# timlod/onset-fingerprinting

Hardware: AMD Instinct MI355X
Metric: frames/sec (1024-pt, hop 256, 48 kHz) detect+FFT+classify at 1/2/4/8 MI355X (higher is better)
Workload: dtype f32

## Files before the change

onset_fingerprinting_amd/csrc/ofp_detect.hip:

```cpp
#include <algorithm>
#include <cstdlib>
#include <cmath>
#include <cstring>
#include <new>
#include <vector>

#include "../../include/ofp_math.h"
#include "ofp_common.h"

#include "ofp_detector.h"

#define OFP_LATENCY_BOUND_KERNEL() __builtin_amdgcn_s_setprio(3)

namespace {

using ofp::align_up;
using ofp::cdiv;

typedef float v2f __attribute__((ext_vector_type(2)));

struct Geom {
    int64_t N;
    int64_t Nm;
    int64_t n_w;
// ... 44 lines not shown
        }
    };
    auto load = [&](float4 (&v)[PB4]) {
#pragma unroll
        for (int i = 0; i < PB4; ++i) v[i] = q[i];
        q += PB4;
        __builtin_amdgcn_sched_barrier(0);
    };
    auto run = [&](const float4 (&v)[PB4]) {
        batch(v);
        __builtin_amdgcn_sched_barrier(0);
    };
    float4 A[PB4], Bv[PB4];
    if (nb >= PB4) {
        load(A);
        nb -= PB4;
        while (nb >= 2 * PB4) {
            load(Bv); run(A);
            load(A); run(Bv);
            nb -= 2 * PB4;
        }
        run(A);
    }
    while (nb > 0) {
        const float4 v = *q++;
        one(v.x); one(v.y); one(v.z); one(v.w);
        --nb;
    }
    ip = reinterpret_cast<const float*>(q);
    for (int r = (int)(n & 3); r > 0; --r) one(*ip++);
}

constexpr int WL_PITCH = 36;
template <class F, class D>
__device__ __forceinline__ void walk_lines_to(const float* in0, const float* ip, int64_t n, F& f, float* tile, float* base, D&& dst_of) {
    const int lane = threadIdx.x & 63;
    const int64_t nb = n >> 5;
    int64_t nbmax = nb;
    for (int o = 32; o > 0; o >>= 1) nbmax = max(nbmax, __shfl_xor(nbmax, o));
    const float4* q = reinterpret_cast<const float4*>(ip);
    float4 A[8], Bv[8];
    auto load = [&](float4 (&v)[8], int64_t b) {
        const bool have = b < nb;
        const float4* const p = have ? q : reinterpret_cast<const float4*>(in0);
#pragma unroll
        for (int i = 0; i < 8; ++i) v[i] = p[i];
        q += have ? 8 : 0;
        __builtin_amdgcn_sched_barrier(0);
    };
    auto run = [&](const float4 (&v)[8], int64_t b) {
        const bool have = b < nb;
        if (have) {
#pragma unroll
            for (int i = 0; i < 8; ++i) {
                float4 o;
                o.x = f(v[i].x); o.y = f(v[i].y); o.z = f(v[i].z); o.w = f(v[i].w);
                *reinterpret_cast<float4*>(&tile[lane * WL_PITCH + 4 * i]) = o;
            }
        }
        __builtin_amdgcn_fence(__ATOMIC_RELEASE, "workgroup");
        __builtin_amdgcn_wave_barrier();
        __builtin_amdgcn_fence(__ATOMIC_ACQUIRE, "workgroup");
        const int64_t my = have ? dst_of(b) : -1;
        const unsigned long long hv = __ballot(my >= 0);
#pragma unroll
        for (int j = 0; j < 8; ++j) {
            const int owner = 8 * j + (lane >> 3);
            const int lo = __shfl((int)my, owner), hi = __shfl((int)(my >> 32), owner);
            if ((hv >> owner) & 1ull) {
                float* dst = base + (((int64_t)hi << 32) | (uint32_t)lo) + 4 * (lane & 7);
                *reinterpret_cast<float4*>(dst) = *reinterpret_cast<const float4*>(&tile[owner * WL_PITCH + 4 * (lane & 7)]);
            }
        }
        __builtin_amdgcn_wave_barrier();
        __builtin_amdgcn_sched_barrier(0);
    };
    load(A, 0);
    int64_t b = 0;
    for (; b + 1 < nbmax; b += 2) {
        load(Bv, b + 1); run(A, b);
        load(A, b + 2); run(Bv, b + 1);
    }
    if (b < nbmax) run(A, b);
}
template <class F>
__device__ __forceinline__ void walk_lines(const float* in0, const float* ip, float* base, int64_t off, int64_t n, F& f, float* tile) {
    walk_lines_to(in0, ip, n, f, tile, base, [off](int64_t b) { return off + 32 * b; });
}

template <int CH, int PB, bool EV, class F>
__device__ __forceinline__ void walk_il(const float* ip, int64_t n, int& rem, F& f) {
    auto one = [&](float x) {
        f(x);
        if (EV && rem >= 0) {
            if (rem == 0) f.event();
// ... 292 lines not shown
template <int W>
__device__ __forceinline__ bool chunk_pass_start(int pass, int64_t k, int64_t sidx, const uint32_t* end_prev,
                                                 uint32_t* end_next, uint32_t* used, bool has_dirty, uint8_t* dirty,
                                                 int* changed, uint32_t (&st)[W]) {
#pragma unroll
    for (int w = 0; w < W; ++w) st[w] = used[sidx + w];
    if (pass == 0) return true;
    uint32_t p[W];
    bool keep = k == 0;
    if (!keep) {
        keep = true;
#pragma unroll
        for (int w = 0; w < W; ++w) {
            p[w] = end_prev[sidx - 2 + w];
            keep = keep && p[w] == st[w];
        }
        if (has_dirty && *dirty != 0) keep = false;
    }
    if (keep) {
        keep_end<W>(end_prev, end_next, sidx);
        return false;
    }
    if (has_dirty) *dirty = 0;
#pragma unroll
    for (int w = 0; w < W; ++w) used[sidx + w] = st[w] = p[w];
    atomicAdd(changed, 1);
    return true;
}

struct ArArgs {
    Geom g;
    const float* xdb;
    float* dif;
    float fa, fr, sa, sr, floor_db;
    int64_t L, W, Wc, Wf, n_chunks;
    int64_t S;
    int lines;
    int through;
};
__device__ __forceinline__ bool chunk_walked(int64_t k, int64_t S, int64_t n_chunks) {
    return k + 1 < min((k / S) * S + S, n_chunks);
}

__global__ __launch_bounds__(64) void k_ar_coarse(ArArgs a, int64_t n_threads, uint32_t* __restrict__ used) {
    OFP_LATENCY_BOUND_KERNEL();
    const int64_t id = (int64_t)blockIdx.x * blockDim.x + threadIdx.x;
    if (id >= n_threads) return;
    const LaneAt ln = lane_planar(id, a.n_chunks, a.g.C);
    const int64_t ws = max<int64_t>(ln.k * a.L - a.W, 0);
    const float* xs = a.xdb + ln.chain * a.g.U;
    ArCoarse cs{a.floor_db, a.floor_db, a.fa, a.fr, a.sa, a.sr};
    if (ws > 0) {
        const int64_t t0 = max<int64_t>(ws - a.Wc, 0);
        if (t0 > 0) cs.yf = cs.ys = xs[t0];
        int norem = -1;
        walk<16, 0, false>(xs + t0, nullptr, ws - t0, norem, cs);
    }
    put_state(used, ln.sidx(a.n_chunks), cs.yf, cs.ys);
}

__global__ __launch_bounds__(64) void k_ar_sym_local(ArArgs a, int64_t n_waves, double* __restrict__ P) {
    OFP_LATENCY_BOUND_KERNEL();
    const int64_t id = blockIdx.x;
    if (id >= n_waves) return;
    const int lane = threadIdx.x;
    const int64_t j = id % a.n_chunks;
    const int64_t chain = id / a.n_chunks;
    const int64_t base = j * a.L;
    const int64_t len = min(a.L, a.g.U - base);
    const float* xs = a.xdb + chain * a.g.U + base;
    const double c = (double)a.sa, q = 1.0 - c;
    double q64 = 1.0, w = c;
    for (int i = 0; i < 64; ++i) {
        q64 *= q;
// ... 71 lines not shown
__global__ __launch_bounds__(64) void k_ar_warm2(ArArgs a, int64_t n_threads, uint32_t* __restrict__ used) {
    OFP_LATENCY_BOUND_KERNEL();
    const int64_t half = (n_threads + 63) / 64;
    const bool fast = blockIdx.x >= half;
    const int64_t id = ((int64_t)blockIdx.x - (fast ? half : 0)) * blockDim.x + threadIdx.x;
    if (id >= n_threads) return;
    const LaneAt ln = lane_planar(id, cdiv(a.n_chunks, a.S), a.g.C);
    const int64_t chain = ln.chain;
    const int64_t k0 = ln.k * a.S;
    const int64_t start = k0 * a.L;
    const float* xs = a.xdb + chain * a.g.U;
    int norem = -1;
    if (!fast) {
        const int64_t ws = max<int64_t>(start - a.W, 0);
        ArOne s{ofp_u2f(used[state_idx(chain, a.n_chunks, k0) + 1]), a.sa, a.sr};
        walk<8, 0, false>(xs + ws, nullptr, start - ws, norem, s);
        put_state(used, state_idx(chain, a.n_chunks, k0) + 1, s.y);
        for (int64_t k = k0 + 1; k < min(k0 + a.S, a.n_chunks); ++k) {
            walk<8, 0, false>(xs + (k - 1) * a.L, nullptr, a.L, norem, s);
            put_state(used, state_idx(chain, a.n_chunks, k) + 1, s.y);
        }
    } else {
        const int64_t ws = max<int64_t>(start - min(a.W, a.Wf), 0);
        ArOne s{a.floor_db, a.fa, a.fr};
        walk<8, 0, false>(xs + ws, nullptr, start - ws, norem, s);
        put_state(used, state_idx(chain, a.n_chunks, k0), s.y);
        for (int64_t k = k0 + 1; k < min(k0 + a.S, a.n_chunks); ++k) {
            walk<8, 0, false>(xs + (k - 1) * a.L, nullptr, a.L, norem, s);
            put_state(used, state_idx(chain, a.n_chunks, k), s.y);
        }
    }
}

template <bool LINES>
__global__ __launch_bounds__(64) void k_ar_warm_both(ArArgs a, int64_t n_threads, uint32_t* __restrict__ used,
                                                     uint32_t* __restrict__ end0) {
    OFP_LATENCY_BOUND_KERNEL();
    __shared__ float tile[LINES ? 64 * WL_PITCH : 1];
    const int64_t id = (int64_t)blockIdx.x * blockDim.x + threadIdx.x;
    const bool live = id < n_threads;
    if (!LINES && !live) return;
    const LaneAt ln = lane_planar(id, cdiv(a.n_chunks, a.S), a.g.C, live);
    const int64_t chain = ln.chain;
    const int64_t k0 = ln.k * a.S;
    const int64_t start = k0 * a.L;
    const float* xs = a.xdb + chain * a.g.U;
    int norem = -1;
    const int64_t ws = max<int64_t>(start - a.W, 0);
    const int64_t s0 = state_idx(chain, a.n_chunks, k0);
    ArStep s{a.floor_db, live ? ofp_u2f(used[s0 + 1]) : 0.0f, a.fa, a.fr, a.sa, a.sr};
    if (live) {
        walk<8, 0, false>(xs + ws, nullptr, start - ws, norem, s);
        put_state(used, s0, s.yf, s.ys);
    }
    float* os = a.dif + chain * a.g.U;
    if (LINES) {
        for (int64_t i = 1; i < a.S; ++i) {
            const int64_t k = k0 + i;
            const bool on = live && k < a.n_chunks;
            walk_lines(a.xdb, xs + (on ? (k - 1) * a.L : 0), a.dif, chain * a.g.U + (on ? (k - 1) * a.L : 0), on ? a.L : 0, s, tile);
            if (on) {
                put_state(used, state_idx(chain, a.n_chunks, k), s.yf, s.ys);
                put_state(end0, (chain * a.n_chunks + k - 1) * 2, s.yf, s.ys);
            }
        }
        return;
    }
    for (int64_t k = k0 + 1; k < min(k0 + a.S, a.n_chunks); ++k) {
        if (a.through) walk<8, 4, false>(xs + (k - 1) * a.L, os + (k - 1) * a.L, a.L, norem, s);
        else walk<8, 0, false>(xs + (k - 1) * a.L, nullptr, a.L, norem, s);
        put_state(used, state_idx(chain, a.n_chunks, k), s.yf, s.ys);
        if (a.through) put_state(end0, (chain * a.n_chunks + k - 1) * 2, s.yf, s.ys);
    }
}

template <bool LINES>
__global__ __launch_bounds__(64) void k_ar_chunk(ArArgs a, int pass, int64_t n_threads,
                                                 const uint32_t* __restrict__ end_prev,
                                                 uint32_t* __restrict__ end_next, uint32_t* __restrict__ used,
                                                 int* changed, const int* gate) {
    OFP_LATENCY_BOUND_KERNEL();
    if (gate && *gate == 0) return;
    __shared__ float tile[LINES ? 64 * WL_PITCH : 1];
    const int64_t id = (int64_t)blockIdx.x * blockDim.x + threadIdx.x;
    bool act = id < n_threads;
    const LaneAt ln = lane_planar(id, a.n_chunks, a.g.C, act);
    const int64_t k = ln.k, chain = ln.chain;
    const int64_t start = k * a.L;
    const int64_t end = min(start + a.L, a.g.U);
    const int64_t sidx = ln.sidx(a.n_chunks);
    if (act && pass == 0 && a.through && chunk_walked(k, a.S, a.n_chunks)) act = false;
    uint32_t st[2] = {0, 0};
    if (act) act = chunk_pass_start<2>(pass, k, sidx, end_prev, end_next, used, false, nullptr, changed, st);
    ArStep s{ofp_u2f(st[0]), ofp_u2f(st[1]), a.fa, a.fr, a.sa, a.sr};
    if (LINES) {
        if (!__any(act)) return;
        walk_lines(a.xdb, a.xdb + chain * a.g.U + start, a.dif, chain * a.g.U + start, act ? end - start : 0, s, tile);
    } else {
        if (!act) return;
        int norem = -1;
        walk<8, 4, false>(a.xdb + chain * a.g.U + start, a.dif + chain * a.g.U + start, end - start, norem, s);
    }
    if (act) put_state(end_next, sidx, s.yf, s.ys);
}

struct MmArgs {
    Geom g;
    const float* rel;
    const float* rel_il;
    const float* rel_warm;
    float* thr_mn;
    float* thr_mx;
    float alpha_min, alpha_max, ialpha_min, ialpha_max, minmin, min0, max0;
    int64_t nb, L, W, n_chunks;
    uint8_t* dirty;
    int64_t n_chains;
    int64_t S;
    int through;
};
constexpr int64_t MM_WARM_FULL = 12288;

__device__ __forceinline__ int64_t mm_block_end(const MmArgs& a, int64_t clip, int c, int C, int64_t start, int& rem) {
    const int64_t m = start - a.g.n_wb;
    int64_t j = 0;
    if (m >= 0) {
        j = m / a.g.B;
        rem = (int)(a.g.B - 1 - (m - j * a.g.B));
    } else {
        rem = (int)min<int64_t>(-m + a.g.B - 1, 0x7fffffff);
    }
// ... 1095 lines not shown
    const int64_t m0 = u0 - g.n_wb;
    if (vec && (m0 >= 0 || m0 + nt <= 0) && (reinterpret_cast<uintptr_t>(rel_out) & 15u) == 0) {
        if (m0 < 0 && !dstw) return;
        float4* d4 = reinterpret_cast<float4*>(m0 < 0 ? dstw + u0 * C : dst + m0 * C);
        const int lc = (C & (C - 1)) == 0 ? 31 - __clz(C) : -1;
        for (int i = threadIdx.x; i < (total >> 2); i += 256) {
            float o[4];
#pragma unroll
            for (int e = 0; e < 4; ++e) {
                const int j = 4 * i + e;
                const int t = lc >= 0 ? j >> lc : j / C, c = j - t * C;
                o[e] = tile[c * S + t];
            }
            d4[i] = make_float4(o[0], o[1], o[2], o[3]);
        }
        return;
    }
    for (int i = threadIdx.x; i < total; i += 256) {
        const int t = i / C, c = i - t * C;
        const int64_t m = u0 + t - g.n_wb;
        if (m >= 0) dst[m * C + c] = tile[c * S + t];
        else if (dstw) dstw[(u0 + t) * C + c] = tile[c * S + t];
    }
}

__global__ __launch_bounds__(256) void k_rel_out(Geom g, float* __restrict__ buf, float* __restrict__ rel_out,
                                                 float floor_db, int TU, uint32_t* __restrict__ sum_max,
                                                 uint32_t* __restrict__ sum_minv, int64_t nb, float* __restrict__ rel_warm,
                                                 int planar, int64_t n_tiles) {
    extern __shared__ float tile[];
    for (int64_t tx = blockIdx.x; tx < n_tiles; tx += gridDim.x) {
        rel_out_tile(g, buf, rel_out, floor_db, TU, sum_max, sum_minv, nb, rel_warm, planar, tx, tile);
        __syncthreads();
    }
}

struct ScanArgs {
    Geom g;
    const float* rel;
    const float* thr_mn;
    const float* thr_mx;
    const float* on_f;
    const float* off_f;
    const double* on_d;
    int manual;
    int64_t nb, n_clips;
    int32_t* first_cross;
    int32_t* last_below;
    uint32_t* vflag;
    const uint32_t* sum_max;
    const uint32_t* sum_minv;
};

__global__ __launch_bounds__(256) void k_block_scan(ScanArgs a) {
    OFP_LATENCY_BOUND_KERNEL();
    const int C = a.g.C, B = a.g.B;
    const int lane = threadIdx.x & 63;
    const int64_t total = a.n_clips * a.nb * C;
    const int64_t wave0 = ((int64_t)blockIdx.x * blockDim.x + threadIdx.x) >> 6;
    const int64_t n_waves = ((int64_t)gridDim.x * blockDim.x) >> 6;
    int64_t j = wave0 % a.nb, chain = wave0 / a.nb;
    const int64_t step_j = n_waves % a.nb, step_chain = n_waves / a.nb;
    for (int64_t id = wave0; id < total; id += n_waves, j += step_j, chain += step_chain) {
        if (j >= a.nb) {
            j -= a.nb;
            chain += 1;
// ... 660 lines not shown
constexpr int64_t state_arrays_bytes(int64_t words) { return 3 * words * 4; }
inline StateArrays state_arrays(uint32_t* base, int64_t words) { return StateArrays{base, base + words, base + 2 * words}; }
constexpr int64_t hp_run_lists_bytes(int64_t n0) { return 2 * n0 * (16 + 4 + 4) + 64; }
inline void hp_run_lists(unsigned char* base, int64_t n0, HpRuns (&rl)[2]) {
    for (int i = 0; i < 2; ++i) {
        rl[i].z = reinterpret_cast<float4*>(base) + i * n0;
        rl[i].grp = reinterpret_cast<int32_t*>(base + n0 * 32) + i * n0;
        rl[i].mask = reinterpret_cast<uint32_t*>(base + n0 * 40) + i * n0;
    }
}

struct Layout {
    Geom g;
    int64_t nb;
    int64_t hp_L, hp_W, hp_chunks, hp_delta;
    int hp_R, hp_S, hp_span;
    bool sm_seg;
    bool merge;
    bool hp_early;
    bool hp_staged;
    int64_t ar_L, ar_W, ar_Wc, ar_Wf, ar_chunks, ar_S;
    bool ar_sym;
    int64_t mm_L, mm_W, mm_chunks, mm_S;
    int tu;
    bool hp_lines;
    bool hp_spread;
    int n_cuts = 0;
    int64_t cuts[16] = {};
    bool ar_through;
    bool ar_lines;
    bool db_sym;
    bool mm_il;
    bool mm_through;
    bool use_sum;
    bool host_verify;
    int hp_group;
    int verify_group;
    int max_passes;
    Stage forced_from;
    bool sm_force_sequential;
    int64_t o_xt, o_xdb, o_dif, o_relw, o_hp_U, o_hp_E, o_hp_sel, o_hp_done, o_hp_M, o_hp_nxt, o_hp_guess, o_hp_ran, o_hp_gs, o_hp_pos, o_hp_mrg, o_hp_runs, o_hp_goff, o_hp_stage_n, o_ar_state, o_ar_P, o_mm_state, o_mm_dirty, o_hp_rounds, o_pass_flags, o_sum,
        o_thr_mn, o_thr_mx, o_first, o_last, o_vflag, o_pc, o_visj, o_vrec, o_nv, o_vtile, o_ltile, o_smseg, o_flags, o_zero, zero_bytes, total;
};

int64_t pick(int64_t user, int64_t dflt) { return user > 0 ? user : dflt; }
int64_t pick_warm(int64_t user, int64_t dflt) { return user > 0 ? user : (user < 0 ? 0 : dflt); }

Layout make_layout(const ofp_detector* d, int64_t n_clips, int64_t N, int64_t warm, bool rel = false) {
    Layout l;
    const auto& p = d->p;
    Geom& g = l.g;
    g.C = p.n_channels;
    g.B = p.block_size;
    g.N = N;
    g.Nm = (N / g.B) * g.B;
    g.n_w = std::max<int64_t>(0, std::min(warm, N));
    g.n_wb = (g.n_w / g.B) * g.B;
    g.U = g.n_wb + g.Nm;
    g.V = g.n_w + g.Nm;
    g.Nv = align_up(g.n_w + N, 4);
    l.nb = g.Nm / g.B;
    const float cmin = std::min(std::min(p.fast_attack, p.fast_release), std::min(p.slow_attack, p.slow_release));
    const double tau = cmin > 0 ? 1.0 / cmin : 1.0;
    const int64_t chains = n_clips * g.C;
    const int64_t share = std::max<int64_t>(1, d->t.concurrent_calls);
    const int64_t cus = std::max<int64_t>(1, (int64_t)d->n_cus / share);
// ... 72 lines not shown
                 (g.U & 31) == 0 &&
                 (g.Nv & 3) == 0 &&
                 (l.hp_L & 31) == 0 &&
                 ((l.hp_L / l.hp_S) & 31) == 0 &&
                 l.hp_L % l.hp_S == 0;
    l.hp_spread = (int64_t)(unsigned)cdiv(chains * l.hp_chunks * (l.hp_R / l.hp_span), HP_CAND_THREADS) <= d->n_cus &&
                  d->t.concurrent_calls <= 1;
    if (l.hp_staged) {
        for (int64_t c = 4096; c < l.hp_W && l.n_cuts < 15; c += (c < 8192 ? 4096 : (c < 40960 ? 8192 : 16384)))
            l.cuts[l.n_cuts++] = c;
        l.cuts[l.n_cuts++] = l.hp_W;
    }
    l.ar_through = d->t.walk_through >= 0 &&
                   l.merge &&
                   l.ar_sym &&
                   (g.U & 3) == 0 &&
                   (l.ar_L & 3) == 0;
    l.ar_lines = d->t.line_stores >= 0 &&
                 (l.ar_through || d->t.line_stores > 0 || chains * l.ar_chunks >= (int64_t)32 * 4 * d->n_cus) &&
                 (g.U & 31) == 0 &&
                 (l.ar_L & 31) == 0;
    l.db_sym = d->t.fuse_db_sums >= 0 &&
               l.ar_sym &&
               p.hp_enabled &&
               (g.U & 3) == 0 &&
               (l.ar_L & 3) == 0;
    l.mm_il = d->t.interleaved >= 0 &&
              d->t.interleaved != 2 &&
              l.merge &&
              rel &&
              !p.manual &&
              (g.C == 4 || g.C == 8 || g.C == 64);
    l.mm_through = l.mm_il && d->t.walk_through >= 0;
    l.use_sum = d->t.scan_skip >= 0 &&
                (g.U & 3) == 0 &&
                (l.tu & 3) == 0 &&
                ((g.n_wb * g.C) & 3) == 0 &&
                (((int64_t)l.tu * g.C) & 3) == 0 &&
                ((g.Nm * g.C) & 3) == 0 &&
                (g.B & 3) == 0 &&
                g.B >= 32;
    l.host_verify = d->t.host_verify > 0;
    l.hp_group = d->t.verify_group > 0 ? (int)std::min<int64_t>(d->t.verify_group, 8) : 0;
    l.verify_group = d->t.verify_group > 0 ? (int)d->t.verify_group : 2;
    l.max_passes = d->t.max_passes;
    l.forced_from = d->t.host_verify == -2 ? HEAD : (d->t.host_verify == -3 ? FOLLOWERS : (d->t.host_verify <= -4 ? TRACKER : END));
    l.sm_force_sequential = d->t.sm_segments == 2;

    int64_t o = 0;
    auto take = [&](int64_t bytes) {
        int64_t r = o;
        o += align_up(bytes, 256);
        return r;
    };
    l.o_xt = take(n_clips * g.C * g.Nv * 4 + 64);
    l.o_xdb = take(n_clips * g.C * g.U * 4 + 64);
    l.o_dif = take(n_clips * g.C * g.U * 4 + 64);
    l.o_relw = take(n_clips * g.C * g.n_wb * 4 + 64);
    {
        const int64_t cc = n_clips * l.hp_chunks * g.C;
        l.o_hp_U = take(cc * (l.hp_R + 1) * 16);
        l.o_hp_E = take(cc * (l.hp_R + 1) * 16);
        l.o_hp_sel = take(cc);
        l.o_hp_done = take(cc * l.hp_S);
        l.o_hp_M = take(cc * l.hp_R * (l.hp_S - 1) * 16 + 16);
        l.o_hp_nxt = take(cc * (l.hp_R + 1));
// ... 158 lines not shown
    template <class T>
    T* at(int64_t off) const { return reinterpret_cast<T*>(ws + off); }
    int64_t chains() const { return a.n_clips * l.g.C; }
    size_t tile_lds() const { return (size_t)l.g.C * (l.tu + 4) * sizeof(float); }
};

bool capturing(hipStream_t stream) {
    hipStreamCaptureStatus cs = hipStreamCaptureStatusNone;
    return hipStreamIsCapturing(stream, &cs) == hipSuccess && cs != hipStreamCaptureStatusNone;
}

int open_call(Call& c, ofp_detector* d, const float* d_x, int64_t n_clips, int64_t N, int64_t warm, float* d_rel,
              ofp_onset* d_records, int64_t cap, int64_t* d_counts, void* d_ws, int64_t ws_bytes, void* stream,
              bool may_capture) {
    OFP_REQUIRE(d && d_counts && d_ws, "ofp_detect_offline: NULL argument");
    OFP_REQUIRE(n_clips >= 1 && N >= 0 && cap >= 0, "ofp_detect_offline: bad sizes");
    OFP_REQUIRE(d_x || N == 0, "ofp_detect_offline: d_x is NULL");
    OFP_REQUIRE(d_records || cap == 0, "ofp_detect_offline: d_records is NULL");
    OFP_REQUIRE(n_clips <= 65535, "ofp_detect_offline: at most 65535 clips per call");
    c.l = make_layout(d, n_clips, N, warm, d_rel != nullptr);
    const Layout& l = c.l;
    if (ws_bytes < l.total)
        return ofp::fail(OFP_ERR_WORKSPACE, "work space %lld < required %lld bytes", (long long)ws_bytes, (long long)l.total);
    c.d = d; c.x = d_x; c.rec = &d->pend;
    c.a = ofp_detect_args{n_clips, N, warm, d_rel, d_records, cap, d_counts, d_ws, ws_bytes};
    c.ws = static_cast<unsigned char*>(d_ws);
    c.stream = (hipStream_t)stream;
    c.timed = !capturing(c.stream);
    OFP_REQUIRE(c.timed || may_capture, "ofp_detect_offline: the stream is capturing; use ofp_detect_offline_enqueue");
    c.ctr = Counters{c.at<int>(l.o_flags), 0, c.stream};
    c.xt = c.at<float>(l.o_xt); c.xdb = c.at<float>(l.o_xdb); c.dif = c.at<float>(l.o_dif); c.rel_warm = c.at<float>(l.o_relw);
    c.sum_max = l.use_sum ? c.at<uint32_t>(l.o_sum) : nullptr;
    c.sum_minv = l.use_sum ? c.sum_max + n_clips * l.nb * l.g.C : nullptr;
    return OFP_OK;
}

template <class F>
auto with_il_channels(int C, F f) {
    if (C == 8) return f(std::integral_constant<int, 8>());
    if (C == 64) return f(std::integral_constant<int, 64>());
    return f(std::integral_constant<int, 4>());
}

int head(Call& c) {
    const Layout& l = c.l;
    const Geom& g = l.g;
    if (c.timed) OFP_HIP(hipEventRecord(c.d->ev[0], c.stream));
    const int64_t n16 = l.zero_bytes / 16;
    hipLaunchKernelGGL(k_zero, dim3((unsigned)cdiv(n16, 256)), dim3(256), 0, c.stream, c.at<uint4>(l.o_zero), n16);
    OFP_LAUNCH_CHECK("k_zero");
    const int64_t n_tiles = cdiv(g.N, l.tu);
    const unsigned gx = (unsigned)std::min<int64_t>(n_tiles, std::max<int64_t>(1, (int64_t)32 * c.d->n_cus / c.a.n_clips));
    hipLaunchKernelGGL(k_transpose_in, dim3(gx, (unsigned)c.a.n_clips), dim3(256), c.tile_lds(), c.stream, c.x, c.xt, g.N,
                       g.C, l.tu, g.n_w, g.Nv, n_tiles);
    OFP_LAUNCH_CHECK("k_transpose_in");
    if (c.timed) OFP_HIP(hipEventRecord(c.d->ev[8], c.stream));
    return OFP_OK;
}

HpCand hp_cand(const Call& c) {
    const Layout& l = c.l;
    HpCand hc;
    hc.st.g = l.g;
    hc.st.xt = c.xt; hc.st.out = c.xdb;
    std::memcpy(hc.st.b, c.d->b, sizeof(hc.st.b));
    std::memcpy(hc.st.a, c.d->a, sizeof(hc.st.a));
// ... 97 lines not shown
    const int* last = nullptr;
    for (int it = 0;;) {
        const int G = l.hp_group > 0 ? l.hp_group : (it == 0 ? 3 : 2);
        int* cnt = nullptr;
        if (int rc = c.ctr.take(2 * G, &cnt)) return rc;
        if (cnt == c.ctr.base + OFP_N_COUNTERS - 16) last = nullptr;
        for (int q = 0; q < G; ++q) {
            iir_round(c, hc, cnt + 2 * q, last);
            last = cnt + 2 * q;
        }
        OFP_LAUNCH_CHECK("k_hp_match / k_hp_resolve / k_hp_run");
        OFP_HIP(hipMemcpyAsync(h_flags, cnt, 2 * G * sizeof(int), hipMemcpyDeviceToHost, c.stream));
        OFP_HIP(hipStreamSynchronize(c.stream));
        int stuck = 0;
        for (int q = 0; q < G; ++q) {
            stuck = h_flags[2 * q] + h_flags[2 * q + 1];
            rec.info[0] += 1;
            rec.info[3] += stuck;
            if (stuck == 0) break;
        }
        it += G;
        if (stuck == 0) break;
        if (l.max_passes > 0 && it > l.max_passes)
            return ofp::fail(OFP_ERR_NOCONVERGE, "hp stage: %d chains still unresolved after %d rounds", stuck, it);
    }
    return OFP_OK;
}

ArArgs ar_args(const Call& c) {
    const Layout& l = c.l;
    const auto& p = c.d->p;
    ArArgs a;
    a.g = l.g;
    a.xdb = c.xdb; a.dif = c.dif;
    a.fa = p.fast_attack; a.fr = p.fast_release; a.sa = p.slow_attack; a.sr = p.slow_release; a.floor_db = p.floor_db;
    a.L = l.ar_L; a.W = l.ar_W; a.Wc = l.ar_Wc; a.Wf = l.ar_Wf; a.n_chunks = l.ar_chunks; a.S = l.ar_S;
    a.through = l.ar_through ? 1 : 0; a.lines = l.ar_lines ? 1 : 0;
    return a;
}

int decibels(Call& c) {
    const Layout& l = c.l;
    const auto& p = c.d->p;
    const int64_t chains = c.chains();
    if (l.db_sym) {
        hipLaunchKernelGGL(k_rect_db_sym, dim3((unsigned)(chains * l.ar_chunks)), dim3(64), 0, c.stream, ar_args(c), c.xdb,
                           chains * l.ar_chunks, c.at<double>(l.o_ar_P));
        OFP_LAUNCH_CHECK("k_rect_db_sym");
    } else {
        const unsigned ew_grid = (unsigned)std::min<int64_t>(cdiv(chains * l.g.U, 256), 256 * 16);
        hipLaunchKernelGGL(k_rect_db, dim3(ew_grid), dim3(256), 0, c.stream, l.g, c.xt, c.xdb, chains, p.hp_enabled ? 0 : 1,
                           p.floor_db);
        OFP_LAUNCH_CHECK("k_rect_db");
    }
    return OFP_OK;
}

int followers(Call& c, bool host_verified) {
    const Layout& l = c.l;
    const ArArgs a = ar_args(c);
    const int64_t chains = c.chains();
    const int64_t nt = chains * l.ar_chunks;
    uint32_t* used = c.at<uint32_t>(l.o_ar_state);
    if (l.ar_sym) {
        double* P = c.at<double>(l.o_ar_P);
        if (!l.db_sym) {
            hipLaunchKernelGGL(k_ar_sym_local, dim3((unsigned)nt), dim3(64), 0, c.stream, a, nt, P);
            OFP_LAUNCH_CHECK("k_ar_sym_local");
        }
        hipLaunchKernelGGL(k_ar_sym_combine, dim3((unsigned)chains), dim3(64), 0, c.stream, a, (const double*)P, used);
        OFP_LAUNCH_CHECK("k_ar_sym_combine");
        const int64_t ntg = chains * cdiv(l.ar_chunks, l.ar_S);
        if (l.merge)
            hipLaunchKernelGGL(l.ar_lines ? k_ar_warm_both<true> : k_ar_warm_both<false>, dim3((unsigned)cdiv(ntg, 64)), dim3(64),
                               0, c.stream, a, ntg, used, state_arrays(used, 2 * nt).endA);
        else
            hipLaunchKernelGGL(k_ar_warm2, dim3(2 * (unsigned)cdiv(ntg, 64)), dim3(64), 0, c.stream, a, ntg, used);
        OFP_LAUNCH_CHECK("k_ar_warm2");
    } else {
        const unsigned grid = (unsigned)cdiv(nt, 64);
        hipLaunchKernelGGL(k_ar_coarse, dim3(grid), dim3(64), 0, c.stream, a, nt, used);
        OFP_LAUNCH_CHECK("k_ar_coarse");
        hipLaunchKernelGGL(k_ar_warm, dim3(grid), dim3(64), 0, c.stream, a, nt, used);
        OFP_LAUNCH_CHECK("k_ar_warm");
    }
    const auto chunk = l.ar_lines ? k_ar_chunk<true> : k_ar_chunk<false>;
    ofp_detect_pending& rec = *c.rec;
    if (!host_verified) {
        rec.ar_nv = l.ar_chunks > 1 ? std::max(2, std::min(AHEAD_MAX_PASSES / 2, c.d->ar_pass_hint)) : 0;
        return run_jacobi_ahead("follower stage", chunk, a, nt, l.ar_chunks, used, c.at<int>(l.o_pass_flags), rec.ar_nv,
                                c.stream);
    }
    return run_jacobi("follower stage", chunk, a, nt, l.ar_chunks, used, c.ctr, c.d->h_flags, l.max_passes, l.verify_group,
                      c.stream, &rec.info[1], &rec.info[3]);
}

int rel_out(Call& c) {
    const Layout& l = c.l;
    const Geom& g = l.g;
    const int64_t n_clips = c.a.n_clips;
    const size_t lds = c.tile_lds() + (l.use_sum ? (size_t)2 * g.C * (l.tu / g.B + 2) * 4 : 0);
    const int64_t n_tiles = cdiv(g.U, l.tu);
    const unsigned gx = (unsigned)std::min<int64_t>(n_tiles, std::max<int64_t>(1, (int64_t)32 * c.d->n_cus / n_clips));
    hipLaunchKernelGGL(k_rel_out, dim3(gx, (unsigned)n_clips), dim3(256), lds, c.stream, g, c.dif, c.a.rel, c.d->p.floor_db,
                       l.tu, c.sum_max, c.sum_minv, l.nb, l.mm_il ? c.rel_warm : nullptr, l.mm_il ? 0 : 1, n_tiles);
    OFP_LAUNCH_CHECK("k_rel_out");
    return OFP_OK;
}

int tracker(Call& c, bool host_verified) {
    const Layout& l = c.l;
    const auto& p = c.d->p;
    ofp_detect_pending& rec = *c.rec;
    if (p.manual) return OFP_OK;
    const int64_t chains = c.chains();
    MmArgs a;
    a.g = l.g;
    a.rel = c.dif; a.rel_il = c.a.rel; a.rel_warm = c.rel_warm;
    a.thr_mn = c.at<float>(l.o_thr_mn); a.thr_mx = c.at<float>(l.o_thr_mx);
    a.alpha_min = p.alpha_min; a.alpha_max = p.alpha_max;
    a.ialpha_min = c.d->ialpha_min; a.ialpha_max = c.d->ialpha_max;
    a.minmin = p.minmin; a.min0 = p.min0; a.max0 = p.max0;
    a.nb = l.nb; a.L = l.mm_L; a.W = l.mm_W; a.n_chunks = l.mm_chunks; a.n_chains = chains; a.S = l.mm_S;
    a.through = l.mm_through ? 1 : 0;
    a.dirty = c.at<uint8_t>(l.o_mm_dirty);
    const int64_t nt = chains * l.mm_chunks;
    uint32_t* used = c.at<uint32_t>(l.o_mm_state);
    const int64_t ntg = chains * cdiv(l.mm_chunks, l.mm_S);
    if (l.mm_il)
        with_il_channels(l.g.C, [&](auto ch) {
            hipLaunchKernelGGL(k_mm_warm_il<decltype(ch)::value>, dim3((unsigned)cdiv(ntg, 64)), dim3(64), 0, c.stream, a, ntg,
                               used, state_arrays(used, 2 * nt).endA);
        });
    else if (l.merge)
        hipLaunchKernelGGL(k_mm_warm_both, dim3((unsigned)cdiv(ntg, 64)), dim3(64), 0, c.stream, a, ntg, used);
    else
        hipLaunchKernelGGL(k_mm_warm2, dim3(2 * (unsigned)cdiv(ntg, 64)), dim3(64), 0, c.stream, a, ntg, used);
    OFP_LAUNCH_CHECK("k_mm_warm2");
    using MmLight = void (*)(const MmArgs&, int64_t, const uint32_t*, uint32_t*, uint32_t*, int*, const int*, hipStream_t);
    const MmLight light_pl = +[](const MmArgs& m, int64_t, const uint32_t* ep, uint32_t* en, uint32_t* u, int* ch, const int* gate,
                                 hipStream_t st) {
        const int64_t n = m.n_chains * m.n_chunks;
        hipLaunchKernelGGL(k_mm_maxpass, dim3((unsigned)cdiv(n, 64)), dim3(64), 0, st, m, n, ep, en, u, ch, gate);
    };
    const MmLight light_il = +[](const MmArgs& m, int64_t, const uint32_t* ep, uint32_t* en, uint32_t* u, int* ch, const int* gate,
                                 hipStream_t st) {
        const int64_t n = m.n_chains * m.n_chunks;
        with_il_channels(m.g.C, [&](auto cc) {
            hipLaunchKernelGGL(k_mm_maxpass_il<decltype(cc)::value>, dim3((unsigned)cdiv(n, 64)), dim3(64), 0, st, m, n, ep, en, u,
                               ch, gate);
        });
// ... 2 lines not shown
    const auto chunk = l.mm_il ? with_il_channels(l.g.C, [](auto ch) { return k_mm_chunk_il<decltype(ch)::value>; })
                               : (l.merge ? k_mm_chunk_both : k_mm_chunk);
    const int64_t n_threads = l.merge ? nt : 2 * 64 * cdiv(nt, 64);
    if (!host_verified) {
        rec.mm_nv = l.mm_chunks > 1 ? std::max(2, std::min(AHEAD_MAX_PASSES / 2, c.d->mm_pass_hint)) : 0;
        return run_jacobi_ahead("tracker stage", chunk, a, n_threads, l.mm_chunks, used,
                                c.at<int>(l.o_pass_flags) + AHEAD_MAX_PASSES, rec.mm_nv, c.stream, light, 2 * nt);
    }
    return run_jacobi("tracker stage", chunk, a, n_threads, l.mm_chunks, used, c.ctr, c.d->h_flags, l.max_passes,
                      l.verify_group, c.stream, &rec.info[2], &rec.info[3], light, 2 * nt);
}

SmArgs sm_args(const Call& c) {
    const Layout& l = c.l;
    SmArgs sm;
    sm.g = l.g;
    sm.nb = l.nb; sm.n_clips = c.a.n_clips; sm.cap = c.a.cap; sm.cooldown = c.d->p.cooldown;
    sm.vis_j = c.at<int32_t>(l.o_visj);
    sm.vfc = c.at<int32_t>(l.o_vrec);
    sm.vlb = sm.vfc + c.a.n_clips * l.nb * l.g.C;
    sm.vpc = sm.vlb + c.a.n_clips * l.nb * l.g.C;
    sm.nv = c.at<int32_t>(l.o_nv);
    sm.records = c.a.records; sm.counts = c.a.counts; sm.clip_base = 0;
    return sm;
}

int crossings(Call& c) {
    const Layout& l = c.l;
    const Geom& g = l.g;
    const int64_t n_clips = c.a.n_clips;
    const int64_t chains = c.chains();
    ScanArgs sa;
    sa.g = g;
    sa.rel = c.dif; sa.thr_mn = c.at<float>(l.o_thr_mn); sa.thr_mx = c.at<float>(l.o_thr_mx);
    sa.on_f = c.d->d_on_f; sa.off_f = c.d->d_off_f; sa.on_d = c.d->d_on_d; sa.manual = c.d->p.manual;
    sa.nb = l.nb; sa.n_clips = n_clips;
    sa.first_cross = c.at<int32_t>(l.o_first); sa.last_below = c.at<int32_t>(l.o_last); sa.vflag = c.at<uint32_t>(l.o_vflag);
    sa.sum_max = c.sum_max; sa.sum_minv = c.sum_minv;
    if (l.mm_il) {
        const unsigned il_grid = (unsigned)std::min<int64_t>(cdiv(n_clips * l.nb, 4), 256 * 32);
        with_il_channels(g.C, [&](auto ch) {
            hipLaunchKernelGGL(k_block_scan_il<decltype(ch)::value>, dim3(il_grid), dim3(256), 0, c.stream, sa, c.a.rel);
        });
    } else {
        const unsigned bs_grid = (unsigned)std::min<int64_t>(cdiv(n_clips * l.nb * g.C, 4), 256 * 32);
        hipLaunchKernelGGL(k_block_scan, dim3(bs_grid), dim3(256), 0, c.stream, sa);
    }
    OFP_LAUNCH_CHECK("k_block_scan");
    const SmArgs sm = sm_args(c);
    VisArgs va;
    va.vflag = sa.vflag; va.fc = sa.first_cross; va.lb = sa.last_below;
    int32_t* pc = c.at<int32_t>(l.o_pc);
    va.pc = pc; va.nb = l.nb; va.C = g.C;
    va.vis_j = const_cast<int32_t*>(sm.vis_j); va.nv = const_cast<int32_t*>(sm.nv);
    va.vfc = const_cast<int32_t*>(sm.vfc); va.vlb = const_cast<int32_t*>(sm.vlb); va.vpc = const_cast<int32_t*>(sm.vpc);
    {
        const int64_t n_lt = cdiv(l.nb, 256);
        int32_t* lt = c.at<int32_t>(l.o_ltile);
        OFP_REQUIRE(n_lt * chains < (1ll << 31), "ofp_detect_offline: %lld block tiles in one call", (long long)(n_lt * chains));
        const dim3 lgrid((unsigned)(n_lt * chains));
        hipLaunchKernelGGL(k_last_clear<false>, lgrid, dim3(64), 0, c.stream, (const int32_t*)sa.last_below, pc, lt, l.nb, g.C, n_lt);
        hipLaunchKernelGGL(k_last_clear_scan, dim3((unsigned)chains), dim3(64), 0, c.stream, lt, n_lt);
        hipLaunchKernelGGL(k_last_clear<true>, lgrid, dim3(64), 0, c.stream, (const int32_t*)sa.last_below, pc, lt, l.nb, g.C, n_lt);
        OFP_LAUNCH_CHECK("k_last_clear");
    }
    const int64_t n_tiles = cdiv(l.nb, 256);
    int32_t* vtile = c.at<int32_t>(l.o_vtile);
// ... 20 lines not shown
    const Layout& l = c.l;
    c.rec->sm_flag = false;
    if (!l.sm_seg) return sequential_machine(c);
    const int64_t n_clips = c.a.n_clips;
    const SmArgs sm = sm_args(c);
    SmSegArgs ss;
    ss.n_seg = cdiv(l.nb, SM_SEG);
    const int64_t words = n_clips * ss.n_seg * 64 * 2;
    ss.used = c.at<int32_t>(l.o_smseg);
    ss.endA = ss.used + words;
    ss.endB = ss.endA + words;
    ss.cnt = ss.endB + words;
    const int tb = std::max(1, std::min(64, 1024 / l.g.C));
    const size_t lds = (size_t)3 * tb * l.g.C * 4 + 64 * 4;
    const dim3 grid((unsigned)ss.n_seg, (unsigned)n_clips);
    constexpr int V = 4;
    int* cnt = nullptr;
    if (int rc = c.ctr.take(V, &cnt)) return rc;
    hipLaunchKernelGGL(k_sm_seg, grid, dim3(64), lds, c.stream, sm, ss, 0, cnt);
    for (int q = 1; q <= V; ++q) hipLaunchKernelGGL(k_sm_seg, grid, dim3(64), lds, c.stream, sm, ss, q, cnt + q - 1);
    hipLaunchKernelGGL(k_sm_offsets, dim3((unsigned)n_clips), dim3(64), 0, c.stream, sm, ss);
    hipLaunchKernelGGL(k_sm_seg, grid, dim3(64), lds, c.stream, sm, ss, -1, cnt);
    OFP_LAUNCH_CHECK("k_sm_seg / k_sm_offsets");
    c.rec->sm_flag = true;
    OFP_HIP(hipMemcpyAsync(c.d->h_flags + 40, cnt + V - 1, sizeof(int), hipMemcpyDeviceToHost, c.stream));
    return OFP_OK;
}

int backtrack(const Call& c) {
    const auto& p = c.d->p;
    if (!(p.backtrack && c.a.cap > 0)) return OFP_OK;
    BtArgs bt;
    bt.g = c.l.g;
    bt.rel = c.dif; bt.rel_il = c.l.mm_il ? c.a.rel : nullptr;
    bt.records = c.a.records; bt.counts = c.a.counts; bt.cap = c.a.cap; bt.n_clips = c.a.n_clips;
    bt.N = p.backtrack_buffer_size; bt.alpha = p.backtrack_alpha; bt.tol = p.backtrack_tol;
    hipLaunchKernelGGL(k_backtrack, dim3((unsigned)cdiv(c.a.n_clips * c.a.cap, 64)), dim3(64), 0, c.stream, bt);
    OFP_LAUNCH_CHECK("k_backtrack");
    return OFP_OK;
}

int run(Call& c, Stage first, Stage last, bool host_verified) {
    ofp_detect_pending& rec = *c.rec;
    rec.valid = false;
    if (first == HEAD) rec.timed = c.timed;
    else c.timed = c.timed && rec.timed;
    rec.empty = c.l.nb == 0;
    if (rec.empty) {
        if (last == END) {
            hipLaunchKernelGGL(k_zero_i64, dim3((unsigned)cdiv(c.a.n_clips, 256)), dim3(256), 0, c.stream, c.a.counts, c.a.n_clips);
            OFP_LAUNCH_CHECK("k_zero_i64");
        }
        return OFP_OK;
    }
    if (first == HEAD) {
        rec.hp_timed = rec.staged = false;
        std::memset(rec.info, 0, sizeof(rec.info));
        if (int rc = head(c)) return rc;
    }
    if (first <= CANDIDATES && last >= CANDIDATES)
        if (int rc = iir_candidates(c)) return rc;
    if (last != END) return OFP_OK;
    rec.ahead = !host_verified;
    rec.hp_rounds = rec.ar_nv = rec.mm_nv = 0;
    hipEvent_t* ev = c.d->ev;
    if (first <= ROUNDS)
        if (int rc = iir_rounds(c, host_verified)) return rc;
// ... 319 lines not shown
```

Before: 215.3 million.

## Write AR detector output directly in interleaved channel layout and add interleaved rel-out pass

The attack/release walk kernels gain an interleaved mode that transposes each 32-sample line through LDS and writes straight into the channel-interleaved rel/rel_warm buffers, rather than into the planar dif buffer. A new k_rel_out_il kernel then applies the linear conversion in place and reduces per-block max/min, replacing the planar tile-based rel_out pass. Downstream scan, backtrack and mm kernels drop their planar dif pointer whenever mm_il is active. The aim is to remove a planar-to-interleaved transpose round trip through memory. The cost is gating on extra geometry and alignment conditions, plus strided LDS reads for the transpose.

```diff
diff --git a/onset_fingerprinting_amd/csrc/ofp_detect.hip b/onset_fingerprinting_amd/csrc/ofp_detect.hip
--- a/onset_fingerprinting_amd/csrc/ofp_detect.hip
+++ b/onset_fingerprinting_amd/csrc/ofp_detect.hip
@@ -100,8 +100,9 @@
 }
 
 constexpr int WL_PITCH = 36;
-template <class F, class D>
-__device__ __forceinline__ void walk_lines_to(const float* in0, const float* ip, int64_t n, F& f, float* tile, float* base, D&& dst_of) {
+template <int IL = 0, class F, class D>
+__device__ __forceinline__ void walk_lines_to(const float* in0, const float* ip, int64_t n, F& f, float* tile, float* base, D&& dst_of,
+                                              float* base_w = nullptr) {
     const int lane = threadIdx.x & 63;
     const int64_t nb = n >> 5;
     int64_t nbmax = nb;
@@ -129,6 +130,27 @@
         __builtin_amdgcn_fence(__ATOMIC_RELEASE, "workgroup");
         __builtin_amdgcn_wave_barrier();
         __builtin_amdgcn_fence(__ATOMIC_ACQUIRE, "workgroup");
+        if constexpr (IL != 0) {
+            constexpr int F4 = 8 * IL;
+            constexpr int Q = IL / 4;
+            const int64_t at = have ? dst_of(b) : 0;
+            const unsigned long long hv = __ballot(have);
+            const int m = lane % F4, t = m / Q, c0 = 4 * (m % Q);
+#pragma unroll
+            for (int j = 0; j < 8; ++j) {
+                const int g0 = (j * (64 / F4) + lane / F4) * IL;
+                const int lo = __shfl((int)at, g0), hi = __shfl((int)(at >> 32), g0);
+                if ((hv >> g0) & 1ull) {
+                    const int64_t enc = ((int64_t)hi << 32) | (uint32_t)lo;
+                    float* dst = (enc < 0 ? base_w + ~enc : base + enc) + 4 * m;
+                    const float* src = &tile[(g0 + c0) * WL_PITCH + t];
+                    *reinterpret_cast<float4*>(dst) = make_float4(src[0], src[WL_PITCH], src[2 * WL_PITCH], src[3 * WL_PITCH]);
+                }
+            }
+            __builtin_amdgcn_wave_barrier();
+            __builtin_amdgcn_sched_barrier(0);
+            return;
+        }
         const int64_t my = have ? dst_of(b) : -1;
         const unsigned long long hv = __ballot(my >= 0);
 #pragma unroll
@@ -487,6 +509,8 @@
     Geom g;
     const float* xdb;
     float* dif;
+    float* rel;
+    float* rel_warm;
     float fa, fr, sa, sr, floor_db;
     int64_t L, W, Wc, Wf, n_chunks;
     int64_t S;
@@ -495,6 +519,10 @@
 };
 __device__ __forceinline__ bool chunk_walked(int64_t k, int64_t S, int64_t n_chunks) {
     return k + 1 < min((k / S) * S + S, n_chunks);
+}
+template <int CH>
+__device__ __forceinline__ int64_t ar_il_dst(const Geom& g, int64_t clip, int64_t u) {
+    return u < g.n_wb ? ~((clip * g.n_wb + u) * CH) : (clip * g.Nm + (u - g.n_wb)) * CH;
 }
 
 __global__ __launch_bounds__(64) void k_ar_coarse(ArArgs a, int64_t n_threads, uint32_t* __restrict__ used) {
@@ -632,7 +660,7 @@
     }
 }
 
-template <bool LINES>
+template <bool LINES, int IL = 0>
 __global__ __launch_bounds__(64) void k_ar_warm_both(ArArgs a, int64_t n_threads, uint32_t* __restrict__ used,
                                                      uint32_t* __restrict__ end0) {
     OFP_LATENCY_BOUND_KERNEL();
@@ -640,7 +668,8 @@
     const int64_t id = (int64_t)blockIdx.x * blockDim.x + threadIdx.x;
     const bool live = id < n_threads;
     if (!LINES && !live) return;
-    const LaneAt ln = lane_planar(id, cdiv(a.n_chunks, a.S), a.g.C, live);
+    const LaneAt ln = IL ? lane_il<IL ? IL : 4>(live ? id : 0, cdiv(a.n_chunks, a.S))
+                         : lane_planar(id, cdiv(a.n_chunks, a.S), a.g.C, live);
     const int64_t chain = ln.chain;
     const int64_t k0 = ln.k * a.S;
     const int64_t start = k0 * a.L;
@@ -658,7 +687,14 @@
         for (int64_t i = 1; i < a.S; ++i) {
             const int64_t k = k0 + i;
             const bool on = live && k < a.n_chunks;
-            walk_lines(a.xdb, xs + (on ? (k - 1) * a.L : 0), a.dif, chain * a.g.U + (on ? (k - 1) * a.L : 0), on ? a.L : 0, s, tile);
+            if constexpr (IL != 0) {
+                const Geom& g = a.g;
+                const int64_t clip = ln.clip, u0 = (k - 1) * a.L;
+                walk_lines_to<IL>(a.xdb, xs + (on ? u0 : 0), on ? a.L : 0, s, tile, a.rel,
+                                  [&](int64_t b) { return ar_il_dst<IL>(g, clip, u0 + 32 * b); }, a.rel_warm);
+            } else {
+                walk_lines(a.xdb, xs + (on ? (k - 1) * a.L : 0), a.dif, chain * a.g.U + (on ? (k - 1) * a.L : 0), on ? a.L : 0, s, tile);
+            }
             if (on) {
                 put_state(used, state_idx(chain, a.n_chunks, k), s.yf, s.ys);
                 put_state(end0, (chain * a.n_chunks + k - 1) * 2, s.yf, s.ys);
@@ -674,7 +710,7 @@
     }
 }
 
-template <bool LINES>
+template <bool LINES, int IL = 0>
 __global__ __launch_bounds__(64) void k_ar_chunk(ArArgs a, int pass, int64_t n_threads,
                                                  const uint32_t* __restrict__ end_prev,
                                                  uint32_t* __restrict__ end_next, uint32_t* __restrict__ used,
@@ -684,7 +720,7 @@
     __shared__ float tile[LINES ? 64 * WL_PITCH : 1];
     const int64_t id = (int64_t)blockIdx.x * blockDim.x + threadIdx.x;
     bool act = id < n_threads;
-    const LaneAt ln = lane_planar(id, a.n_chunks, a.g.C, act);
+    const LaneAt ln = IL ? lane_il<IL ? IL : 4>(act ? id : 0, a.n_chunks) : lane_planar(id, a.n_chunks, a.g.C, act);
     const int64_t k = ln.k, chain = ln.chain;
     const int64_t start = k * a.L;
     const int64_t end = min(start + a.L, a.g.U);
@@ -695,7 +731,16 @@
     ArStep s{ofp_u2f(st[0]), ofp_u2f(st[1]), a.fa, a.fr, a.sa, a.sr};
     if (LINES) {
         if (!__any(act)) return;
-        walk_lines(a.xdb, a.xdb + chain * a.g.U + start, a.dif, chain * a.g.U + start, act ? end - start : 0, s, tile);
+        if constexpr (IL != 0) {
+            const Geom& g = a.g;
+            const int64_t clip = ln.clip;
+            const int lane0 = (threadIdx.x & 63) & ~(IL - 1);
+            const bool with = ((__ballot(act) >> lane0) & ((1ull << IL) - 1)) != 0;
+            walk_lines_to<IL>(a.xdb, a.xdb + chain * a.g.U + start, with ? end - start : 0, s, tile, a.rel,
+                              [&](int64_t b) { return ar_il_dst<IL>(g, clip, start + 32 * b); }, a.rel_warm);
+        } else {
+            walk_lines(a.xdb, a.xdb + chain * a.g.U + start, a.dif, chain * a.g.U + start, act ? end - start : 0, s, tile);
+        }
     } else {
         if (!act) return;
         int norem = -1;
@@ -1857,6 +1902,57 @@
     for (int64_t tx = blockIdx.x; tx < n_tiles; tx += gridDim.x) {
         rel_out_tile(g, buf, rel_out, floor_db, TU, sum_max, sum_minv, nb, rel_warm, planar, tx, tile);
         __syncthreads();
+    }
+}
+
+template <int CH>
+__global__ __launch_bounds__(256) void k_rel_out_il(Geom g, float* __restrict__ rel, float* __restrict__ rel_warm, float floor_db,
+                                                    uint32_t* __restrict__ sum_max, uint32_t* __restrict__ sum_minv,
+                                                    int64_t nb, int64_t n_wu) {
+    const int lane = threadIdx.x & 63;
+    const int wave = __builtin_amdgcn_readfirstlane(threadIdx.x >> 6);
+    const int64_t clip = blockIdx.y;
+    const int n4 = g.B * (CH / 4);
+    for (int64_t j = (int64_t)blockIdx.x * 4 + wave; j < n_wu + nb; j += (int64_t)gridDim.x * 4) {
+        const bool in_main = j >= n_wu;
+        float4* const p = in_main ? reinterpret_cast<float4*>(rel + (clip * g.Nm + (j - n_wu) * g.B) * CH)
+                               : reinterpret_cast<float4*>(rel_warm + (clip * g.n_wb + j * g.B) * CH);
+        float4 hi = make_float4(0.0f, 0.0f, 0.0f, 0.0f);
+        const float inf = __builtin_inff();
+        float4 lo = make_float4(inf, inf, inf, inf);
+        auto one = [&](int i, float4 v) {
+            v.x = ofp_rel_linear(v.x, floor_db);
+            v.y = ofp_rel_linear(v.y, floor_db);
+            v.z = ofp_rel_linear(v.z, floor_db);
+            v.w = ofp_rel_linear(v.w, floor_db);
+            p[i] = v;
+            hi.x = fmaxf(hi.x, v.x); hi.y = fmaxf(hi.y, v.y); hi.z = fmaxf(hi.z, v.z); hi.w = fmaxf(hi.w, v.w);
+            lo.x = fminf(lo.x, v.x); lo.y = fminf(lo.y, v.y); lo.z = fminf(lo.z, v.z); lo.w = fminf(lo.w, v.w);
+        };
+        int i = lane;
+        for (; i + 192 < n4; i += 256) {
+            const float4 v0 = p[i], v1 = p[i + 64], v2 = p[i + 128], v3 = p[i + 192];
+            __builtin_amdgcn_sched_barrier(0);
+            one(i, v0);
+            one(i + 64, v1);
+            one(i + 128, v2);
+            one(i + 192, v3);
+        }
+        for (; i < n4; i += 64) one(i, p[i]);
+        if (sum_max == nullptr || !in_main) continue;
+#pragma unroll
+        for (int o = 32; o >= CH / 4; o >>= 1) {
+            hi.x = fmaxf(hi.x, __shfl_xor(hi.x, o)); hi.y = fmaxf(hi.y, __shfl_xor(hi.y, o));
+            hi.z = fmaxf(hi.z, __shfl_xor(hi.z, o)); hi.w = fmaxf(hi.w, __shfl_xor(hi.w, o));
+            lo.x = fminf(lo.x, __shfl_xor(lo.x, o)); lo.y = fminf(lo.y, __shfl_xor(lo.y, o));
+            lo.z = fminf(lo.z, __shfl_xor(lo.z, o)); lo.w = fminf(lo.w, __shfl_xor(lo.w, o));
+        }
+        if (lane < CH / 4) {
+            auto minv = [&](float v) { return 0x7f800000u - ofp_f2u(v >= 0.0f ? v : inf); };
+            const int64_t at = (clip * nb + (j - n_wu)) * CH + 4 * lane;
+            *reinterpret_cast<uint4*>(sum_max + at) = make_uint4(ofp_f2u(hi.x), ofp_f2u(hi.y), ofp_f2u(hi.z), ofp_f2u(hi.w));
+            *reinterpret_cast<uint4*>(sum_minv + at) = make_uint4(minv(lo.x), minv(lo.y), minv(lo.z), minv(lo.w));
+        }
     }
 }
 
@@ -2583,6 +2679,7 @@
     bool db_sym;
     bool mm_il;
     bool mm_through;
+    bool ar_il;
     bool use_sum;
     bool host_verify;
     int hp_group;
@@ -2721,6 +2818,13 @@
               !p.manual &&
               (g.C == 4 || g.C == 8 || g.C == 64);
     l.mm_through = l.mm_il && d->t.walk_through >= 0;
+    l.ar_il = l.ar_lines &&
+              l.ar_through &&
+              l.mm_il &&
+              (g.C == 4 || g.C == 8) &&
+              (g.n_wb & 31) == 0 &&
+              (g.Nm & 31) == 0 &&
+              (int64_t)g.B * g.C >= 256;
     l.use_sum = d->t.scan_skip >= 0 &&
                 (g.U & 3) == 0 &&
                 (l.tu & 3) == 0 &&
@@ -2945,6 +3049,7 @@
     c.xt = c.at<float>(l.o_xt); c.xdb = c.at<float>(l.o_xdb); c.dif = c.at<float>(l.o_dif); c.rel_warm = c.at<float>(l.o_relw);
     c.sum_max = l.use_sum ? c.at<uint32_t>(l.o_sum) : nullptr;
     c.sum_minv = l.use_sum ? c.sum_max + n_clips * l.nb * l.g.C : nullptr;
+    if ((reinterpret_cast<uintptr_t>(d_rel) & 15u) != 0) c.l.ar_il = false;
     return OFP_OK;
 }
 
@@ -3108,7 +3213,7 @@
     const auto& p = c.d->p;
     ArArgs a;
     a.g = l.g;
-    a.xdb = c.xdb; a.dif = c.dif;
+    a.xdb = c.xdb; a.dif = c.dif; a.rel = c.a.rel; a.rel_warm = c.rel_warm;
     a.fa = p.fast_attack; a.fr = p.fast_release; a.sa = p.slow_attack; a.sr = p.slow_release; a.floor_db = p.floor_db;
     a.L = l.ar_L; a.W = l.ar_W; a.Wc = l.ar_Wc; a.Wf = l.ar_Wf; a.n_chunks = l.ar_chunks; a.S = l.ar_S;
     a.through = l.ar_through ? 1 : 0; a.lines = l.ar_lines ? 1 : 0;
@@ -3148,8 +3253,9 @@
         OFP_LAUNCH_CHECK("k_ar_sym_combine");
         const int64_t ntg = chains * cdiv(l.ar_chunks, l.ar_S);
         if (l.merge)
-            hipLaunchKernelGGL(l.ar_lines ? k_ar_warm_both<true> : k_ar_warm_both<false>, dim3((unsigned)cdiv(ntg, 64)), dim3(64),
-                               0, c.stream, a, ntg, used, state_arrays(used, 2 * nt).endA);
+            hipLaunchKernelGGL(l.ar_il ? (l.g.C == 8 ? k_ar_warm_both<true, 8> : k_ar_warm_both<true, 4>)
+                                       : (l.ar_lines ? k_ar_warm_both<true> : k_ar_warm_both<false>),
+                               dim3((unsigned)cdiv(ntg, 64)), dim3(64), 0, c.stream, a, ntg, used, state_arrays(used, 2 * nt).endA);
         else
             hipLaunchKernelGGL(k_ar_warm2, dim3(2 * (unsigned)cdiv(ntg, 64)), dim3(64), 0, c.stream, a, ntg, used);
         OFP_LAUNCH_CHECK("k_ar_warm2");
@@ -3160,7 +3266,8 @@
         hipLaunchKernelGGL(k_ar_warm, dim3(grid), dim3(64), 0, c.stream, a, nt, used);
         OFP_LAUNCH_CHECK("k_ar_warm");
     }
-    const auto chunk = l.ar_lines ? k_ar_chunk<true> : k_ar_chunk<false>;
+    const auto chunk = l.ar_il ? (l.g.C == 8 ? k_ar_chunk<true, 8> : k_ar_chunk<true, 4>)
+                               : (l.ar_lines ? k_ar_chunk<true> : k_ar_chunk<false>);
     ofp_detect_pending& rec = *c.rec;
     if (!host_verified) {
         rec.ar_nv = l.ar_chunks > 1 ? std::max(2, std::min(AHEAD_MAX_PASSES / 2, c.d->ar_pass_hint)) : 0;
@@ -3175,6 +3282,14 @@
     const Layout& l = c.l;
     const Geom& g = l.g;
     const int64_t n_clips = c.a.n_clips;
+    if (l.ar_il) {
+        const int64_t n_wu = g.n_wb / g.B;
+        const unsigned gx = (unsigned)std::min<int64_t>(cdiv(n_wu + l.nb, 4), std::max<int64_t>(1, (int64_t)16 * c.d->n_cus / n_clips));
+        hipLaunchKernelGGL(g.C == 8 ? k_rel_out_il<8> : k_rel_out_il<4>, dim3(gx, (unsigned)n_clips), dim3(256), 0, c.stream, g,
+                           c.a.rel, c.rel_warm, c.d->p.floor_db, c.sum_max, c.sum_minv, l.nb, n_wu);
+        OFP_LAUNCH_CHECK("k_rel_out_il");
+        return OFP_OK;
+    }
     const size_t lds = c.tile_lds() + (l.use_sum ? (size_t)2 * g.C * (l.tu / g.B + 2) * 4 : 0);
     const int64_t n_tiles = cdiv(g.U, l.tu);
     const unsigned gx = (unsigned)std::min<int64_t>(n_tiles, std::max<int64_t>(1, (int64_t)32 * c.d->n_cus / n_clips));
@@ -3192,7 +3307,7 @@
     const int64_t chains = c.chains();
     MmArgs a;
     a.g = l.g;
-    a.rel = c.dif; a.rel_il = c.a.rel; a.rel_warm = c.rel_warm;
+    a.rel = l.mm_il ? nullptr : c.dif; a.rel_il = c.a.rel; a.rel_warm = c.rel_warm;
     a.thr_mn = c.at<float>(l.o_thr_mn); a.thr_mx = c.at<float>(l.o_thr_mx);
     a.alpha_min = p.alpha_min; a.alpha_max = p.alpha_max;
     a.ialpha_min = c.d->ialpha_min; a.ialpha_max = c.d->ialpha_max;
@@ -3261,7 +3376,7 @@
     const int64_t chains = c.chains();
     ScanArgs sa;
     sa.g = g;
-    sa.rel = c.dif; sa.thr_mn = c.at<float>(l.o_thr_mn); sa.thr_mx = c.at<float>(l.o_thr_mx);
+    sa.rel = l.mm_il ? nullptr : c.dif; sa.thr_mn = c.at<float>(l.o_thr_mn); sa.thr_mx = c.at<float>(l.o_thr_mx);
     sa.on_f = c.d->d_on_f; sa.off_f = c.d->d_off_f; sa.on_d = c.d->d_on_d; sa.manual = c.d->p.manual;
     sa.nb = l.nb; sa.n_clips = n_clips;
     sa.first_cross = c.at<int32_t>(l.o_first); sa.last_below = c.at<int32_t>(l.o_last); sa.vflag = c.at<uint32_t>(l.o_vflag);
@@ -3348,7 +3463,7 @@
     if (!(p.backtrack && c.a.cap > 0)) return OFP_OK;
     BtArgs bt;
     bt.g = c.l.g;
-    bt.rel = c.dif; bt.rel_il = c.l.mm_il ? c.a.rel : nullptr;
+    bt.rel = c.l.mm_il ? nullptr : c.dif; bt.rel_il = c.l.mm_il ? c.a.rel : nullptr;
     bt.records = c.a.records; bt.counts = c.a.counts; bt.cap = c.a.cap; bt.n_clips = c.a.n_clips;
     bt.N = p.backtrack_buffer_size; bt.alpha = p.backtrack_alpha; bt.tol = p.backtrack_tol;
     hipLaunchKernelGGL(k_backtrack, dim3((unsigned)cdiv(c.a.n_clips * c.a.cap, 64)), dim3(64), 0, c.stream, bt);
```

New measurement: 229.5 million, median of 6. 1.07x the previous value.
